# Ledicia/Molecular-Dynamics-Simulation---Lennard-Jones-monoatomic-fluid

Measured on AMD Instinct MI355X. Metric: md_steps_per_sec_n262144_fp64, higher is better.
Workload: dtype f64

## Files before the change

molecular-dynamics-simulation---lennard-jones-monoatomic-fluid_amd/csrc/ljmd_common.cpp:

```cpp
#include "ljmd_common.h"
#include "ljmd_internal.h"

#include <algorithm>
#include <cstdio>
#include <cstring>
#include <limits>

namespace ljmdh {

using namespace ljmdk;

thread_local std::string g_last_error = "";

int failv(std::string *handle_err, int code, const char *fmt, va_list ap)
{
    char buf[512];
    vsnprintf(buf, sizeof buf, fmt, ap);
    g_last_error = buf;
    if (handle_err) *handle_err = buf;
    return code;
}

int check_sim_params(const char *who, int n, double box_length, double dt, double rc)
{
// ... 13 lines not shown
        return fail(nullptr, LJMD_ERR_NO_DEVICE, "%s: no HIP device available (this library has no CPU path)", who);
    if (device < 0 || device >= ndev)
        return fail(nullptr, LJMD_ERR_INVALID_ARG, "%s: device %d out of range (0..%d)", who, device, ndev - 1);
    return LJMD_OK;
}

SimParams derive_params(int n, double box_length, double dt, double rc)
{
    SimParams p;
    p.L = box_length;
    p.invL = 1.0 / box_length;
    p.volume = box_length * box_length * box_length;
    p.rc = rc;
    p.rc2 = rc * rc;
    p.dt = dt;
    p.dt_half = 0.5 * dt;
    p.dt_sq_half = p.dt_half * dt;
    {
        const double npd = (double)n;
        const double rc3 = (rc * rc) * rc;
        const double rc6 = ((rc * rc) * (rc * rc)) * (rc * rc);
        const double tf = 8.0 * kPi * (npd * npd) / (p.volume * rc3);
        p.tail_e = tf * ((1.0 / (3.0 * rc6)) - 1.0) / 3.0;
        p.tail_d = 2.0 * tf * (-2.0 / (3.0 * rc6) + 1.0);
        p.tail_dd = 2.0 * tf * (26.0 / (3.0 * rc6) - 7.0);
    }
    return p;
}

Knobs read_knobs()
{
    auto flag = [](const char *name, bool dflt) { return env_int(name, dflt ? 1 : 0) != 0; };
    auto is = [](const char *name, const char *value) {
        const char *v = std::getenv(name);
        return v && std::strcmp(v, value) == 0;
    };
    auto opt_int = [](const char *name) -> std::optional<int> {
        const char *v = std::getenv(name);
        if (v && *v) return std::atoi(v);
        return std::nullopt;
    };
    Knobs k;
    k.sort = flag("LJMD_SORT", k.sort);
    k.force_generic = flag("LJMD_FORCE_GENERIC", k.force_generic);
    k.force_collectives = flag("LJMD_FORCE_COLLECTIVES", k.force_collectives);
    k.fuse = flag("LJMD_FUSE", k.fuse);
    k.fuse_tail = flag("LJMD_FUSE_TAIL", k.fuse_tail);
    k.fuse_defer_record = flag("LJMD_FUSE_DEFER_RECORD", k.fuse_defer_record);
    k.xcd_remap = std::max(0, env_int("LJMD_N3_XCD_REMAP", k.xcd_remap));
    k.inject_failure_at_step = env_int("LJMD_INJECT_FAILURE_AT_STEP", k.inject_failure_at_step);
    k.exchange_alltoall = is("LJMD_FORCE_EXCHANGE", "alltoall");
    k.resort_every = opt_int("LJMD_RESORT_EVERY");
    k.kd_sort_cub = is("LJMD_KD_SORT", "cub");
    k.n3_row_tiles = env_int("LJMD_N3_ROW_TILES", k.n3_row_tiles);
    k.n3_wg_waves = env_int("LJMD_N3_WG_WAVES", k.n3_wg_waves);
    k.slab_budget_gb = std::max(1, env_int("LJMD_SLAB_BUDGET_GB", k.slab_budget_gb));
    k.n3_both_ties = flag("LJMD_N3_BOTH_TIES", k.n3_both_ties);
    k.n3_min_n = env_int("LJMD_N3_MIN_N", k.n3_min_n);
    k.n3 = flag("LJMD_N3", k.n3);
    k.n3_target_waves = opt_int("LJMD_N3_TARGET_WAVES");
    k.n3_clusters = flag("LJMD_N3_CLUSTERS", k.n3_clusters);
    k.n3_pertile = flag("LJMD_N3_PERTILE", k.n3_pertile);
    k.reduce_split = opt_int("LJMD_REDUCE_SPLIT");
    if (k.reduce_split) k.reduce_split = std::max(0, *k.reduce_split);
    k.walk_chunk = opt_int("LJMD_WALK_CHUNK");
    k.vanhove_chunk = opt_int("LJMD_VANHOVE_CHUNK");
    k.fp32_far_stream = flag("LJMD_FP32_FAR_STREAM", k.fp32_far_stream);
    k.fp32_vfar = flag("LJMD_FP32_VFAR", k.fp32_vfar);
    {
        const char *rs = std::getenv("LJMD_FP32_SPLIT");
        if (rs && *rs) k.fp32_split = std::max(0.0, std::atof(rs));
    }
    k.overlap_exchange = flag("LJMD_OVERLAP_EXCHANGE", k.overlap_exchange);
    k.migrate_blocks = is("LJMD_MIGRATE_DEAL", "blocks");
    {
        const char *xm = std::getenv("LJMD_MULTI_EXCHANGE");
        k.multi_exchange = xm ? xm : "";
    }
    k.multi_migrate_every = std::max(0, env_int("LJMD_MULTI_MIGRATE_EVERY", k.multi_migrate_every));
    k.multi_threads = flag("LJMD_MULTI_THREADS", k.multi_threads);
    k.batch_group_streams = !is("LJMD_BATCH_GROUP_STREAMS", "0");
    return k;
}

void scalars_from_sums(double s12, double s6, double kx, double ky, double kz, double te, double td, double tdd,
                       double *epot, double *ekin, double *d_epot, double *dd_epot)
{
    if (epot) *epot = 4.0 * (s12 - s6) + te;
    if (d_epot) *d_epot = 24.0 * (-2.0 * s12 + s6) + td;
    if (dd_epot) *dd_epot = 24.0 * (26.0 * s12 - 7.0 * s6) + tdd;
    if (ekin) *ekin = 0.5 * (kx + ky + kz);
}

namespace {
void neg192(uint64_t (&x)[3])
{
    x[0] = ~x[0]; x[1] = ~x[1]; x[2] = ~x[2];
    const uint64_t one[3] = {1, 0, 0};
    add192(x, one);
}

void scale192(uint64_t (&x)[3], uint64_t k)
{
    unsigned __int128 carry = 0;
    for (int w = 0; w < 3; ++w) {
        const unsigned __int128 p = (unsigned __int128)x[w] * k + carry;
// ... 50 lines not shown
```

molecular-dynamics-simulation---lennard-jones-monoatomic-fluid_amd/csrc/ljmd_common.h:

```cpp
#ifndef LJMD_COMMON_H
#define LJMD_COMMON_H

#include "ljmd.h"

#include <hip/hip_runtime.h>

#include <cstdarg>
#include <cstddef>
#include <cstdint>
#include <cstdlib>
#include <optional>
#include <string>

namespace ljmdh {

extern thread_local std::string g_last_error;

constexpr double kPi = 3.1415926535897932384626433832795;

int failv(std::string *handle_err, int code, const char *fmt, va_list ap);

inline int fail(std::nullptr_t, int code, const char *fmt, ...)
{
    va_list ap;
// ... 20 lines not shown
    failv(h ? &const_cast<H *>(h)->err : nullptr, code, fmt, ap);
    va_end(ap);
    return code;
}

#define LJMD_HIP(h, call)                                                                   \
    do {                                                                                    \
        hipError_t e_ = (call);                                                             \
        if (e_ != hipSuccess)                                                               \
            return ljmdh::fail((h), LJMD_ERR_HIP, "%s failed: %s (%s:%d)", #call,           \
                               hipGetErrorString(e_), __FILE__, __LINE__);                  \
    } while (0)

#define LJMD_TRY(expr)                      \
    do {                                    \
        const int rc__ = (expr);            \
        if (rc__ != LJMD_OK) return rc__;   \
    } while (0)

inline int env_int(const char *name, int dflt)
{
    const char *v = std::getenv(name);
    return (v && *v) ? std::atoi(v) : dflt;
}

int check_sim_params(const char *who, int n, double box_length, double dt, double rc);

int probe_device(int device, const char *who);

struct SimParams {
    double L = 0, invL = 0, volume = 0, rc = 0, rc2 = 0, dt = 0, dt_half = 0, dt_sq_half = 0;
    double tail_e = 0, tail_d = 0, tail_dd = 0;
};
SimParams derive_params(int n, double box_length, double dt, double rc);

void scalars_from_sums(double s12, double s6, double kx, double ky, double kz, double te, double td, double tdd,
                       double *epot, double *ekin, double *d_epot, double *dd_epot);

void scalars_from_exact_sums(const uint64_t (&ordered)[5][3], double te, double td, double tdd, bool have_e, bool have_k,
                             double *epot, double *ekin, double *d_epot, double *dd_epot);

struct Knobs {
    bool sort = true;
    bool force_generic = false;
    bool force_collectives = false;
    bool fuse = true;
    bool fuse_tail = true;
    bool fuse_defer_record = true;
    int xcd_remap = 4;
    int inject_failure_at_step = -1;
    bool exchange_alltoall = false;
    std::optional<int> resort_every;
    bool kd_sort_cub = false;
    int n3_row_tiles = 0;
    int n3_wg_waves = 0;
    int slab_budget_gb = 64;
    bool n3_both_ties = true;
    int n3_min_n = 4096;
    bool n3 = true;
    std::optional<int> n3_target_waves;
    bool n3_clusters = true;
    bool n3_pertile = true;
    std::optional<int> reduce_split;
    std::optional<int> walk_chunk;
    std::optional<int> vanhove_chunk;
    bool fp32_far_stream = true;
    bool fp32_vfar = true;
    double fp32_split = 5.0;
    bool overlap_exchange = true;
    bool migrate_blocks = false;
    std::string multi_exchange;
    int multi_migrate_every = 2000;
    bool multi_threads = true;
    bool batch_group_streams = true;
};
Knobs read_knobs();

}
#endif
```

molecular-dynamics-simulation---lennard-jones-monoatomic-fluid_amd/csrc/ljmd_engine.cpp:

```cpp
#include "ljmd_engine.h"

namespace ljmdh {

bool fast_path_ok(const ljmd_t *h) { return h->plan.rc_allows_fast && h->positions_compact && !h->knobs.force_generic; }

double *wg_part_now(ljmd_t *h) { return h->d_wg_part + (h->plan.fuse_tail ? (size_t)h->fold_parity * h->wg_part_stride : 0); }

PairArgs pair_args(ljmd_t *h, bool fast)
{
    PairArgs a;
    a.pos = h->d_pos;
    a.slab = h->d_slab;
    a.wg_part = wg_part_now(h);
    a.mask = h->d_mask;
    a.bbox = h->d_bbox;
    a.inline_mask = (fast && h->plan.fuse_tail && !h->plan.use_n3) ? 1 : 0;
    a.rc2_skin = h->rc2 * (1.0 + 1e-10);
    a.n = h->n;
    a.S = h->plan.S;
    a.P = h->plan.P;
    a.G = h->G;
    a.rank = h->rank;
    a.TB = h->plan.TB;
    a.T = h->plan.T;
// ... 97 lines not shown
{
    ReduceArgs a;
    a.slab = h->d_slab;
    a.slab_j = n3 ? h->d_slab_j : nullptr;
    a.flag_j = n3 ? h->d_flag_j : nullptr;
    a.slab_j2 = (n3 && h->mode == LJMD_PRECISION_FP32_FORCE) ? reinterpret_cast<const float *>(h->d_slab_j2) : nullptr;
    a.flag_j2 = (n3 && h->mode == LJMD_PRECISION_FP32_FORCE) ? h->d_flag_j2 : nullptr;
    a.fpart = h->d_fpart;
    a.nslab = nslab;
    a.P = h->plan.P;
    a.G = h->G;
    a.rank = h->rank;
    a.TB = h->plan.TB;
    a.CS = h->plan.CS;
    a.CS2 = h->plan.CS2;
    a.RT = h->plan.rt;
    a.partial = h->d_red_part;
    a.c_split = h->plan.split_s1;
    a.j_split = h->plan.split_j1;
    return a;
}

FinalizeArgs finalize_args(ljmd_t *h, int n_wg, bool with_ke, double pair_scale)
{
    FinalizeArgs a;
    a.pair_scale = pair_scale;
    a.wg_part = wg_part_now(h);
    a.ke_part = h->d_ke_part;
    a.ke_tile = nullptr;
    a.ring = h->d_ring;
    a.ring_pos = h->d_ring_pos;
    a.n_wg = n_wg;
    a.n_ke = with_ke ? h->plan.n_ke : 0;
    a.ring_cap = kRingCap;
    return a;
}

EventSet *next_events(ljmd_t *h)
{
    if (!h->profiling || h->ev_used >= (size_t)kMaxProfiledLaunches) return nullptr;
    if (h->ev_used == h->ev_pool.size()) {
        EventSet q;
        for (auto &e : q.e)
            if (hipEventCreate(&e) != hipSuccess) return nullptr;
        h->ev_pool.push_back(q);
    }
    EventSet *q = &h->ev_pool[h->ev_used++];
    q->has_pos_x = q->has_force_x = false;
    return q;
}

int resort(ljmd_t *h, bool with_accel)
{
    if (!launch_kd_finish || !launch_gather_state)
        return fail(h, LJMD_ERR_HIP, "resort: this build holds no launch_kd_finish / launch_gather_state (ljmd_sort.h)");
    const int levels = (int)h->plan.kd_level_nseg.size(), from = h->plan.kd_finish_from;
    int *cur = h->d_idx, *nxt = h->d_idx2;
    LJMD_HIP(h, launch_iota(cur, h->plan.P, h->stream));
    if (from > 0) LJMD_HIP(h, launch_iota(nxt, h->plan.P, h->stream));
    for (int l = 0; l < from; ++l) {
        const double *axis = own_block(h) + (size_t)h->kd_axis[l] * h->plan.P;
        LJMD_HIP(h, kd_level(h->d_cub, h->cub_bytes, axis, h->L, h->d_kd_keys, h->d_kd_keys2, cur, nxt, h->plan.S,
                             h->plan.kd_level_nseg[l], h->d_kd_offsets + h->plan.kd_level_off[l], h->stream));
        std::swap(cur, nxt);
    }
    for (int l = from; l < levels; l += kKdFinishMaxLevels) {
        KdFinishArgs ka;
        ka.pos = own_block(h);
        ka.P = h->plan.P;
        ka.scale = (double)(1u << kCoordBits) / h->L;
        ka.idx_in = ka.idx_out = cur;
        ka.offsets = h->d_kd_offsets;
        ka.nlevels = std::min(kKdFinishMaxLevels, levels - l);
        for (int k = 0; k < ka.nlevels; ++k) {
            ka.nseg[k] = h->plan.kd_level_nseg[l + k];
            ka.off[k] = (int)h->plan.kd_level_off[l + k];
            ka.axis[k] = h->kd_axis[l + k];
        }
        LJMD_HIP(h, launch_kd_finish(ka, h->stream));
    }
    GatherStateArgs g;
    double *sets[4] = {own_block(h), h->d_ru, h->d_v, with_accel ? h->d_a : nullptr};
    double *outs[4] = {h->d_tmp3, h->d_ru2, h->d_v2, h->d_a2};
    for (int k = 0; k < 4; ++k) {
        g.src[k] = sets[k];
        g.dst[k] = outs[k];
    }
    g.perm = h->d_perm;
    g.perm_out = h->d_perm2;
    g.idx = cur;
    g.P = h->plan.P;
    LJMD_HIP(h, launch_gather_state(g, h->stream));
    LJMD_HIP(h, hipMemcpyAsync(own_block(h), h->d_tmp3, 3 * (size_t)h->plan.P * sizeof(double), hipMemcpyDeviceToDevice,
                               h->stream));
    std::swap(h->d_ru, h->d_ru2);
    std::swap(h->d_v, h->d_v2);
    if (with_accel) std::swap(h->d_a, h->d_a2);
    std::swap(h->d_perm, h->d_perm2);
    h->perm_dirty = true;
    h->steps_since_sort = 0;
    return LJMD_OK;
}

int refresh_perm(ljmd_t *h)
{
    if (!h->perm_dirty) return LJMD_OK;
    LJMD_HIP(h, hipMemcpyAsync(h->h_perm.data(), h->d_perm, (size_t)h->plan.P * sizeof(int), hipMemcpyDeviceToHost,
                               h->stream));
    LJMD_HIP(h, hipStreamSynchronize(h->stream));
    h->perm_dirty = false;
    return LJMD_OK;
}

bool use_comm_stream(const ljmd_t *h) { return h->knobs.overlap_exchange && h->comm_stream != nullptr; }
// ... 363 lines not shown
```

molecular-dynamics-simulation---lennard-jones-monoatomic-fluid_amd/csrc/ljmd_engine.h:

```cpp
#ifndef LJMD_ENGINE_H
#define LJMD_ENGINE_H

#include "ljmd_common.h"

#include <rccl/rccl.h>

#include <algorithm>
#include <cmath>
#include <cstdio>
#include <cstring>
#include <limits>
#include <mutex>
#include <vector>

#include "ljmd_internal.h"
#include "ljmd_resident.h"
#include "ljmd_sort.h"

using namespace ljmdk;

namespace ljmdh {

constexpr unsigned kRingCap = 4096;
constexpr int kTargetWorkgroups = 2048;
constexpr int kXcdMinGroups = 256;
constexpr int kMixedMinN = 16384;
constexpr long kN3ItemsFor4 = 6000;
constexpr long kN3ItemsFor2 = 1000;
constexpr long kN3LargeItems = 131072;
constexpr int kN3MidTargetItems = 32768;
constexpr int kBothTiesMaxGroups = 128;
constexpr int kFuseTailMaxRowTiles = 2;
constexpr int kFuseTailMaxN = 20000;
constexpr int kReduceSplitMinN = 131072;
constexpr int kReduceSplitShare = 8;
constexpr int kMaxProfiledLaunches = 4096;
constexpr int kEventsPerLaunch = 9;

struct EventSet {
    hipEvent_t e[kEventsPerLaunch];
    bool has_pos_x = false, has_force_x = false;
};

struct LaunchPlan {
    int S = 0, P = 0;
    int TB = 0, T = 0, W = 0;
    bool rc_allows_fast = false;
    bool sort_enabled = true;
    int resort_every = 20;
    std::vector<int> kd_level_nseg;
    std::vector<size_t> kd_level_off;
    std::vector<int> kd_offsets;
    int kd_finish_from = 0;
    int nslab_g = 1, chunk_g = 0;
    int nslab_t = 1, chunk_t = 0;
    bool use_n3 = false;
    int wg_waves = 1;
    bool both_ties = false;
    int uchunk = 0;
    int CS = 0, CS2 = 0, j_by_group = 0;
    int NG = 0, NGo = 0, Dmax = 0, nslab_n = 1, dchunk = 0;
    int rt = kRowTiles;
    bool fuse_tail = false;
    int split_s1 = 0, split_j1 = 0;
    int nslab_max = 1, n_wg_max = 0;
    int n_ke = 0;
};

int plan_engine(const SimParams &sim, int n, int n_ranks, int precision_mode, const Knobs &k, LaunchPlan *out);

}

struct ljmd_multi;

using namespace ljmdh;

struct ljmd : ljmdh::SimParams {
    ljmd_multi *multi = nullptr;
    bool poisoned = false;
    int inject_failure_at = -1;
    int n = 0, rank = 0, G = 1, device = 0, mode = 0;
    ljmdh::Knobs knobs;
    ljmdh::LaunchPlan plan;
    bool tail_on = true;
    bool positions_compact = false;
    bool positions_wide = false;
    bool have_state = false, have_accel = false;
    int steps_since_sort = 0;

    hipStream_t stream = nullptr;
    ncclComm_t comm = nullptr;
    hipStream_t comm_stream = nullptr;
    hipEvent_t ev_pos_ready = nullptr, ev_gather_done = nullptr;
    bool gather_done_for_step = false;
    double *d_pos = nullptr;
    double *d_ru = nullptr, *d_v = nullptr, *d_a = nullptr;
    double *d_slab = nullptr;
    double *d_wg_part = nullptr;
    double *d_fold = nullptr;
    unsigned *d_ticket = nullptr;
    bool want_energy = true;
    int kick_hint = -1;
    bool next_drift_hint = false;
    bool reduce_deferred = false, deferred_n3 = false;
    int deferred_nslab = 0;
    bool drift_prefused = false;
    double *d_ke_tile = nullptr;
    bool boxes_valid = false;
    double *d_ke_part = nullptr;
    double *d_ring = nullptr;
    int rec_stride = kPartialStride;
    __int128 *d_fslab = nullptr;
    unsigned *d_fflag = nullptr;
    int64_t *d_fblk = nullptr;
    int64_t *d_frec = nullptr;
    bool pending_energy = true;
    unsigned *d_ring_pos = nullptr;
    double *d_bbox = nullptr;
    uint64_t *d_mask = nullptr;
    double *d_pos_tc = nullptr;
    unsigned *d_desc = nullptr;
    unsigned *d_desc_far = nullptr;
    float *d_desc2 = nullptr;
    int *d_idx = nullptr, *d_idx2 = nullptr, *d_perm = nullptr, *d_perm2 = nullptr;
    double *d_tmp3 = nullptr;
    double *d_ru2 = nullptr, *d_v2 = nullptr, *d_a2 = nullptr;
    void *d_cub = nullptr;
    size_t cub_bytes = 0;
    std::vector<int> kd_axis;
    int *d_kd_offsets = nullptr;
    unsigned long long *d_kd_keys = nullptr, *d_kd_keys2 = nullptr;

    unsigned ring_consumed = 0;
    unsigned ring_issued = 0;
    bool fold_pending = false;
    ljmdk::FinalizeArgs pending_fold{};
    int fold_parity = 0;
    size_t wg_part_stride = 0;
    double *d_slab_j = nullptr;
    unsigned char *d_flag_j = nullptr;
    double *d_red_part = nullptr;
    hipStream_t side_stream = nullptr;
    hipEvent_t ev_side_go = nullptr, ev_side_done = nullptr;
    uint64_t *d_mask_far = nullptr;
    double *d_slab_j2 = nullptr;
    unsigned char *d_flag_j2 = nullptr;
    double *d_fpart = nullptr, *d_frecv = nullptr;
    double *d_fall = nullptr;
    bool forces_pending = false;
    bool external_force_exchange = false;
    int pending_n_wg = 0;
    double pending_scale = 0.5;

    double *h_stage = nullptr;
    double *h_ring = nullptr;
    std::vector<int> h_perm;
    bool perm_dirty = false;

    hipStream_t far_stream = nullptr;
    hipEvent_t ev_far_go = nullptr, ev_far_done = nullptr;
    hipStream_t copy_stream = nullptr;
    hipEvent_t ev_snap_ready = nullptr, ev_snap_done = nullptr;
    double *d_snap = nullptr, *h_snap = nullptr;
    int *d_snap_perm = nullptr, *h_snap_perm = nullptr;
    bool snap_in_flight = false;
    bool snap_ready = false;

    int *d_gid0 = nullptr;
    std::vector<int> h_gid0;
    bool migrated = false;
    double *d_mig = nullptr;
    int *d_mig_idx = nullptr, *d_mig_idx2 = nullptr;
    unsigned long long *d_mig_keys = nullptr, *d_mig_keys2 = nullptr;
    int *d_mig_offsets = nullptr;
    void *d_mig_cub = nullptr;
    size_t mig_cub_bytes = 0;
    std::vector<int> mig_level_nseg, mig_axis;
    std::vector<size_t> mig_level_off;
    double mig_ext[3] = {0, 0, 0};
    int32_t migrations = 0;

    ljmdr::RdfState rdf;
    ljmdt::TcfState tcf;
// ... 59 lines not shown
```

molecular-dynamics-simulation---lennard-jones-monoatomic-fluid_amd/csrc/ljmd_plan.cpp:

```cpp
#include "ljmd_engine.h"

namespace ljmdh {

namespace {
int rt_align(int uchunk, int rt)
{
    int m = 1;
    while ((m * uchunk) % rt != 0) ++m;
    return m;
}
}

int plan_engine(const SimParams &sim, int n, int n_ranks, int precision_mode, const Knobs &k, LaunchPlan *out)
{
    LaunchPlan p;
    p.S = n / n_ranks;
    p.P = ((p.S + kSlotAlign - 1) / kSlotAlign) * kSlotAlign;
    p.TB = p.P / kTile;
    p.T = n_ranks * p.TB;
    p.W = (p.T + 63) / 64;
    p.rc_allows_fast = sim.rc <= (1.0 - 1e-9) * 0.5 * sim.L;
    p.sort_enabled = k.sort && n >= 1024;
    p.resort_every = std::max(1, k.resort_every.value_or(n >= 1000000 ? 5 : n >= 131072 ? 10 : n > 40000 ? 20
                                                              : n > kFuseTailMaxN ? 50 : 200));
    {
        const int tiles = (p.S + kTile - 1) / kTile;
        std::vector<int> bounds = {0, tiles};
        while (true) {
            bool any = false;
            for (size_t j = 0; j + 1 < bounds.size(); ++j) any = any || (bounds[j + 1] - bounds[j] > 1);
            if (!any) break;
            p.kd_level_off.push_back(p.kd_offsets.size());
            p.kd_level_nseg.push_back((int)bounds.size() - 1);
            for (int b : bounds) p.kd_offsets.push_back(std::min(b * kTile, p.S));
            std::vector<int> next;
            for (size_t j = 0; j + 1 < bounds.size(); ++j) {
                next.push_back(bounds[j]);
                const int t = bounds[j + 1] - bounds[j];
                if (t > 1) next.push_back(bounds[j] + (t + 1) / 2);
            }
            next.push_back(tiles);
            bounds.swap(next);
        }
        const int levels = (int)p.kd_level_nseg.size();
        p.kd_finish_from = levels;
        for (int l = levels - 1; l >= 0 && !k.kd_sort_cub; --l) {
            int largest = 0;
            for (int j = 0; j < p.kd_level_nseg[l]; ++j)
                largest = std::max(largest, p.kd_offsets[p.kd_level_off[l] + j + 1] - p.kd_offsets[p.kd_level_off[l] + j]);
            if (largest > kKdFinishCap) break;
            p.kd_finish_from = l;
        }
    }

    const int row_blocks = p.P / kBlock;
    {
        int ns = (kTargetWorkgroups + row_blocks - 1) / row_blocks;
        ns = std::max(1, std::min(ns, (n + 63) / 64));
        p.chunk_g = ((n + ns - 1) / ns + 7) / 8 * 8;
        p.nslab_g = (n + p.chunk_g - 1) / p.chunk_g;
    }
    {
        int ns = (kTargetWorkgroups + row_blocks - 1) / row_blocks;
        ns = std::max(1, std::min(ns, p.T));
        p.chunk_t = (p.T + ns - 1) / ns;
        p.nslab_t = (p.T + p.chunk_t - 1) / p.chunk_t;
    }
    {
        const bool mixed_mode = precision_mode == LJMD_PRECISION_FP32_FORCE;
        int rt = k.n3_row_tiles;
        if (mixed_mode) rt = kRowTiles;
        if (rt != 1 && rt != 2 && rt != kRowTiles) {
            auto items = [&](int cand) { const long ngo = p.TB / cand; return ngo * ((long)n_ranks * ngo / 2 + 1); };
            rt = items(kRowTiles) >= kN3ItemsFor4 ? kRowTiles : items(2) >= kN3ItemsFor2 ? 2 : 1;
        }
        p.rt = rt;
        p.NGo = p.TB / rt;
        p.NG = n_ranks * p.NGo;
        p.Dmax = p.NG / 2;
        int wg = k.n3_wg_waves;
        if (wg != 1 && wg != 2 && wg != 4) {
            const double budget = 1e9 * k.slab_budget_gb;
            const double full = (double)p.T * (n_ranks > 1 ? p.NGo : p.Dmax + 1) * 3.0 * kTile * sizeof(double);
            wg = full <= budget ? 1 : full <= 2.0 * budget ? 2 : 4;
        }
        if (rt != kRowTiles || p.NGo < 16 * wg) wg = 1;
        p.wg_waves = wg;
        p.both_ties = wg == 1 && n_ranks == 1 && !mixed_mode && p.NG <= kBothTiesMaxGroups && k.n3_both_ties;
        p.j_by_group = (n_ranks > 1 || p.NG % wg != 0) ? 1 : 0;
        p.CS = p.j_by_group ? (p.NGo + wg - 1) / wg : (p.Dmax + wg - 1) / wg + 1;
        p.CS2 = n_ranks > 1 ? p.NGo : p.Dmax + 1;
        p.use_n3 = k.n3 && n >= k.n3_min_n && (n_ranks == 1 || p.rc_allows_fast) &&
                   precision_mode != LJMD_PRECISION_FP64_REPRODUCIBLE;
        const int n_off = p.Dmax + p.wg_waves;
        const int n_units = n_off * rt;
        const bool plenty = (long)p.NGo * n_off >= kN3LargeItems || n_ranks > 1;
        const int target_waves = std::max(1, k.n3_target_waves.value_or(plenty ? 131072 : kN3MidTargetItems));
        const int ns_wanted = (target_waves + p.NGo - 1) / p.NGo;
        int ns = std::max(1, std::min(ns_wanted, n_off));
        const bool small_single = n_ranks == 1 && n <= kFuseTailMaxN && rt <= kFuseTailMaxRowTiles;
        const int ns_cap = small_single ? std::max(1, kDirectFoldMax / std::max(1, p.NGo)) : n_units;
        ns = std::min(ns, ns_cap);
        p.dchunk = (n_off + ns - 1) / ns;
        p.uchunk = p.dchunk * rt;
// ... 33 lines not shown
```

molecular-dynamics-simulation---lennard-jones-monoatomic-fluid_amd/csrc/ljmd_sort.h:

```cpp
#ifndef LJMD_SORT_H
#define LJMD_SORT_H

#include <hip/hip_runtime.h>

namespace ljmdk {

constexpr int kCoordBits = 24;

constexpr int kKdFinishCap = 4096;
constexpr int kKdFinishMaxLevels = 6;
constexpr int kKdFinishBlock = 1024;

struct KdFinishArgs {
    const double *pos = nullptr;
    int P = 0;
    double scale = 0.0;
    const int *idx_in = nullptr;
    int *idx_out = nullptr;
    const int *offsets = nullptr;
    int nlevels = 0;
    int nseg[kKdFinishMaxLevels] = {};
    int off[kKdFinishMaxLevels] = {};
    int axis[kKdFinishMaxLevels] = {};
};

struct GatherStateArgs {
    const double *src[4] = {};
    double *dst[4] = {};
    const int *perm = nullptr;
    int *perm_out = nullptr;
    const int *idx = nullptr;
    int P = 0;
};

__attribute__((weak)) hipError_t launch_kd_finish(const KdFinishArgs &a, hipStream_t s);
__attribute__((weak)) hipError_t launch_gather_state(const GatherStateArgs &a, hipStream_t s);

}
#endif
```

molecular-dynamics-simulation---lennard-jones-monoatomic-fluid_amd/csrc/ljmd_sort.hip:

```cpp
#include <hip/hip_runtime.h>
#include <hipcub/hipcub.hpp>

#include "ljmd_internal.h"
#include "ljmd_sort.h"

namespace ljmdk {

__global__ __launch_bounds__(kBlock) void gather_state_kernel(GatherStateArgs g)
{
    const int i = blockIdx.x * kBlock + threadIdx.x;
    if (i >= g.P) return;
    const int s = g.idx[i];
#pragma unroll
    for (int q = 0; q < 4; ++q) {
        if (g.src[q] == nullptr) continue;
#pragma unroll
        for (int k = 0; k < 3; ++k) g.dst[q][(size_t)k * g.P + i] = g.src[q][(size_t)k * g.P + s];
    }
    g.perm_out[i] = g.perm[s];
}


__device__ __forceinline__ unsigned long long kd_quant(double coord, double scale)
{
    const double x = coord * scale;
    return (unsigned long long)fmin(fmax(x, 0.0), (double)((1u << kCoordBits) - 1));
}

__global__ __launch_bounds__(kBlock) void kd_keys_kernel(const double *coord, const int *idx, unsigned long long *keys,
                                                         const int *seg_offsets, int nseg, int S, double scale)
{
    const int i = blockIdx.x * kBlock + threadIdx.x;
    if (i >= S) return;
    int lo = 0, hi = nseg;
    while (hi - lo > 1) {
        const int mid = (lo + hi) >> 1;
        if (seg_offsets[mid] <= i) lo = mid; else hi = mid;
    }
    keys[i] = ((unsigned long long)lo << kCoordBits) | kd_quant(coord[idx[i]], scale);
}

__global__ __launch_bounds__(kBlock) void iota_kernel(int *idx, int P)
{
    const int i = blockIdx.x * kBlock + threadIdx.x;
    if (i < P) idx[i] = i;
}

size_t kd_temp_bytes(int count)
{
    size_t bytes = 0;
    (void)hipcub::DeviceRadixSort::SortPairs(nullptr, bytes, (const unsigned long long *)nullptr,
                                             (unsigned long long *)nullptr, (const int *)nullptr, (int *)nullptr,
                                             count, 0, 64, nullptr);
    return bytes;
}

hipError_t launch_iota(int *idx, int P, hipStream_t s)
{
    hipLaunchKernelGGL(iota_kernel, dim3((P + kBlock - 1) / kBlock), dim3(kBlock), 0, s, idx, P);
    return hipGetLastError();
}

hipError_t kd_level(void *temp, size_t temp_bytes, const double *coord_axis, double L, unsigned long long *keys,
                    unsigned long long *keys_out, int *idx, int *idx_out, int S, int nseg, const int *seg_offsets,
                    hipStream_t s)
{
    hipLaunchKernelGGL(kd_keys_kernel, dim3((S + kBlock - 1) / kBlock), dim3(kBlock), 0, s, coord_axis, idx, keys,
                       seg_offsets, nseg, S, (double)(1u << kCoordBits) / L);
    hipError_t e = hipGetLastError();
    if (e != hipSuccess) return e;
    int segbits = 1;
    while ((1 << segbits) < nseg) ++segbits;
    return hipcub::DeviceRadixSort::SortPairs(temp, temp_bytes, keys, keys_out, idx, idx_out, S, 0,
                                              kCoordBits + segbits, s);
}


__device__ __forceinline__ int last_at_most(const int *b, int n, int x)
{
    int lo = 0, hi = n;
    while (hi - lo > 1) {
        const int mid = (lo + hi) >> 1;
        if (b[mid] <= x) lo = mid; else hi = mid;
    }
    return lo;
}

__device__ __forceinline__ void order_pair(unsigned long long &x, unsigned long long &y, bool up)
{
    if ((x > y) == up) {
        const unsigned long long t = x;
        x = y;
        y = t;
    }
}

__global__ __launch_bounds__(kKdFinishBlock) void kd_finish_kernel(KdFinishArgs a)
{
    constexpr int kMaxSub = kKdFinishCap / kTile;
    __shared__ unsigned long long s_word[kKdFinishCap];
    __shared__ int s_idx[kKdFinishCap];
    __shared__ int s_bound[kKdFinishMaxLevels][kMaxSub + 1];
    __shared__ int s_first[kKdFinishMaxLevels], s_last[kKdFinishMaxLevels];
    const int tid = threadIdx.x;
    const int lo = a.offsets[a.off[0] + blockIdx.x], len = a.offsets[a.off[0] + blockIdx.x + 1] - lo;
    if (len <= 0 || len > kKdFinishCap) return;
    int npad = kTile;
    while (npad < len) npad <<= 1;
    for (int p = tid; p < len; p += kKdFinishBlock) s_idx[p] = a.idx_in[lo + p];
    if (tid < kKdFinishMaxLevels) s_first[tid] = s_last[tid] = 0;
    __syncthreads();
    for (int l = 0; l < a.nlevels; ++l)
        for (int j = tid; j <= a.nseg[l]; j += kKdFinishBlock) {
            const int b = a.offsets[a.off[l] + j];
            if (b == lo) s_first[l] = j;
            if (b == lo + len) s_last[l] = j;
        }
    __syncthreads();
    for (int l = 0; l < a.nlevels; ++l) {
        const int nsub = min(s_last[l] - s_first[l], kMaxSub);
        if (tid <= nsub) s_bound[l][tid] = a.offsets[a.off[l] + s_first[l] + tid] - lo;
    }
    __syncthreads();
    for (int l = 0; l < a.nlevels; ++l) {
        const int nsub = min(s_last[l] - s_first[l], kMaxSub);
        const double *coord = a.pos + (size_t)a.axis[l] * a.P;
        for (int p = tid; p < npad; p += kKdFinishBlock) {
            unsigned long long w = ~0ull;
            if (p < len) {
                const unsigned home = l == 0 ? (unsigned)p : (unsigned)(s_word[p] & 0xffffu);
                const int sub = last_at_most(s_bound[l], nsub, p);
                w = ((unsigned long long)sub << 56) | (kd_quant(coord[s_idx[home]], a.scale) << 32) |
                    ((unsigned long long)p << 16) | home;
            }
            s_word[p] = w;
        }
        __syncthreads();
        for (int k = 2; k <= npad; k <<= 1) {
            int j = k >> 1;
            for (; j >= 2; j >>= 2) {
                const int h = j >> 1;
                for (int t = tid; t < (npad >> 2); t += kKdFinishBlock) {
                    const int i = ((t & ~(h - 1)) << 2) | (t & (h - 1));
                    const bool up = (i & k) == 0;
                    unsigned long long w0 = s_word[i], w1 = s_word[i | h], w2 = s_word[i | j], w3 = s_word[i | j | h];
                    order_pair(w0, w2, up);
                    order_pair(w1, w3, up);
                    order_pair(w0, w1, up);
                    order_pair(w2, w3, up);
                    s_word[i] = w0;
                    s_word[i | h] = w1;
                    s_word[i | j] = w2;
                    s_word[i | j | h] = w3;
                }
                __syncthreads();
            }
            if (j == 1) {
                for (int t = tid; t < (npad >> 1); t += kKdFinishBlock) {
                    const int i = t << 1;
                    unsigned long long w0 = s_word[i], w1 = s_word[i | 1];
                    order_pair(w0, w1, (i & k) == 0);
                    s_word[i] = w0;
                    s_word[i | 1] = w1;
                }
                __syncthreads();
            }
        }
    }
    for (int p = tid; p < len; p += kKdFinishBlock) a.idx_out[lo + p] = s_idx[s_word[p] & 0xffffu];
}

hipError_t launch_kd_finish(const KdFinishArgs &a, hipStream_t s)
{
    if (a.nlevels < 1 || a.nlevels > kKdFinishMaxLevels) return hipErrorInvalidValue;
    hipLaunchKernelGGL(kd_finish_kernel, dim3(a.nseg[0]), dim3(kKdFinishBlock), 0, s, a);
    return hipGetLastError();
}

__global__ __launch_bounds__(kBlock) void iota_blocked_kernel(int *idx, int n, int S, int P)
{
    const int k = blockIdx.x * kBlock + threadIdx.x;
    if (k < n) idx[k] = (k / S) * P + k % S;
}

__global__ __launch_bounds__(kBlock) void kd_keys_blocked_kernel(const double *pos, int axis, int P, const int *idx,
                                                                 unsigned long long *keys, const int *seg_offsets, int nseg,
                                                                 int n, double scale)
{
    const int i = blockIdx.x * kBlock + threadIdx.x;
    if (i >= n) return;
    int lo = 0, hi = nseg;
    while (hi - lo > 1) {
        const int mid = (lo + hi) >> 1;
        if (seg_offsets[mid] <= i) lo = mid; else hi = mid;
    }
    const int st = idx[i], g = st / P, sl = st - g * P;
    keys[i] = ((unsigned long long)lo << kCoordBits) | kd_quant(pos[(size_t)g * 3 * P + (size_t)axis * P + sl], scale);
}

__global__ __launch_bounds__(kBlock) void migrate_pack_kernel(const double *ru, const double *v, const double *a,
                                                              const int *perm, const int *gid0, double *block, int S, int P)
{
    const int s = blockIdx.x * kBlock + threadIdx.x;
    if (s >= P) return;
#pragma unroll
    for (int k = 0; k < 3; ++k) {
        block[(size_t)k * P + s] = ru[(size_t)k * P + s];
        block[(size_t)(3 + k) * P + s] = v[(size_t)k * P + s];
        block[(size_t)(6 + k) * P + s] = a[(size_t)k * P + s];
    }
    const int o = perm[s];
    block[(size_t)9 * P + s] = (s < S && o < S) ? (double)gid0[o] : -1.0;
}

__global__ __launch_bounds__(kBlock) void migrate_select_kernel(const double *pos_all, const double *mig_all, const int *mine,
                                                                double *new_pos, double *ru, double *v, double *a, int *gid0,
                                                                int S, int P)
{
    const int j = blockIdx.x * kBlock + threadIdx.x;
    if (j >= P) return;
    if (j >= S) {
#pragma unroll
        for (int k = 0; k < 3; ++k) {
            new_pos[(size_t)k * P + j] = __builtin_nan("");
            ru[(size_t)k * P + j] = __builtin_nan("");
            v[(size_t)k * P + j] = 0.0;
            a[(size_t)k * P + j] = 0.0;
        }
        gid0[j] = -1;
// ... 70 lines not shown
```

molecular-dynamics-simulation---lennard-jones-monoatomic-fluid_amd/csrc/ljmd_storage.cpp:

```cpp
#include "ljmd_engine.h"

namespace ljmdh {

int allocate_engine(ljmd_t *h)
{
    const bool mixed = h->mode == LJMD_PRECISION_FP32_FORCE;
    const std::vector<int> &kd = h->plan.kd_offsets;
    LJMD_HIP(h, hipSetDevice(h->device));
    LJMD_HIP(h, hipStreamCreateWithFlags(&h->stream, hipStreamNonBlocking));
    const size_t P3 = 3 * (size_t)h->plan.P * sizeof(double);
    LJMD_HIP(h, hipMalloc(&h->d_pos, P3 * h->G));
    LJMD_HIP(h, hipMalloc(&h->d_ru, P3));
    LJMD_HIP(h, hipMalloc(&h->d_v, P3));
    LJMD_HIP(h, hipMalloc(&h->d_a, P3));
    LJMD_HIP(h, hipMalloc(&h->d_tmp3, P3));
    if (h->plan.sort_enabled) {
        LJMD_HIP(h, hipMalloc(&h->d_ru2, P3));
        LJMD_HIP(h, hipMalloc(&h->d_v2, P3));
        LJMD_HIP(h, hipMalloc(&h->d_a2, P3));
    }
    LJMD_HIP(h, hipMalloc(&h->d_slab, P3 * h->plan.nslab_max));
    h->wg_part_stride = 2 * (size_t)h->plan.n_wg_max;
    LJMD_HIP(h, hipMalloc(&h->d_wg_part, (h->plan.fuse_tail ? 2 : 1) * h->wg_part_stride * sizeof(double)));
    if (h->plan.use_n3) {
// ... 13 lines not shown
        LJMD_HIP(h, hipStreamCreateWithPriority(&h->side_stream, hipStreamNonBlocking, least));
        LJMD_HIP(h, hipEventCreateWithFlags(&h->ev_side_go, hipEventDisableTiming));
        LJMD_HIP(h, hipEventCreateWithFlags(&h->ev_side_done, hipEventDisableTiming));
    }
    if (mixed && h->knobs.fp32_far_stream) {
        LJMD_HIP(h, hipStreamCreateWithFlags(&h->far_stream, hipStreamNonBlocking));
        LJMD_HIP(h, hipEventCreateWithFlags(&h->ev_far_go, hipEventDisableTiming));
        LJMD_HIP(h, hipEventCreateWithFlags(&h->ev_far_done, hipEventDisableTiming));
    }
    if (mixed) {
        LJMD_HIP(h, hipMalloc(&h->d_mask_far, (size_t)h->plan.TB * h->plan.W * sizeof(uint64_t)));
        LJMD_HIP(h, hipMalloc(&h->d_desc_far, (size_t)h->plan.NGo * h->plan.T * sizeof(unsigned)));
        const size_t n_blk2 = (size_t)h->plan.T * h->plan.CS2;
        LJMD_HIP(h, hipMalloc(&h->d_slab_j2, n_blk2 * 3 * kTile * sizeof(float)));
        LJMD_HIP(h, hipMalloc(&h->d_flag_j2, n_blk2));
        LJMD_HIP(h, hipMemsetAsync(h->d_flag_j2, 0, n_blk2, h->stream));
    }
    LJMD_HIP(h, hipMalloc(&h->d_fpart, P3 * (needs_force_exchange(h) ? h->G : 1)));
    if (needs_force_exchange(h)) LJMD_HIP(h, hipMalloc(&h->d_frecv, P3));
    if (needs_force_exchange(h) && h->knobs.exchange_alltoall) LJMD_HIP(h, hipMalloc(&h->d_fall, P3 * h->G));
    LJMD_HIP(h, hipMalloc(&h->d_ke_part, 3 * (size_t)h->plan.n_ke * sizeof(double)));
    LJMD_HIP(h, hipMalloc(&h->d_fold, 2 * (size_t)kFoldBlocks * sizeof(double)));
    LJMD_HIP(h, hipMalloc(&h->d_ticket, sizeof(unsigned)));
    LJMD_HIP(h, hipMemsetAsync(h->d_ticket, 0, sizeof(unsigned), h->stream));
    if (h->plan.fuse_tail) {
        LJMD_HIP(h, hipMalloc(&h->d_ke_tile, 2 * 3 * (size_t)h->plan.T * sizeof(double)));
        LJMD_HIP(h, hipMemsetAsync(h->d_ke_tile, 0, 2 * 3 * (size_t)h->plan.T * sizeof(double), h->stream));
    }
    if (reproducible(h)) {
        h->rec_stride = kExactWords;
        LJMD_HIP(h, hipMalloc(&h->d_fslab, (size_t)h->plan.nslab_t * kFixedQuantities * h->plan.P * sizeof(__int128)));
        LJMD_HIP(h, hipMalloc(&h->d_fflag, (size_t)h->plan.nslab_t * h->plan.TB * sizeof(unsigned)));
        LJMD_HIP(h, hipMalloc(&h->d_fblk, (size_t)(h->plan.P / kBlock) * kExactWords * sizeof(int64_t)));
        LJMD_HIP(h, hipMalloc(&h->d_frec, kExactWords * sizeof(int64_t)));
    }
    LJMD_HIP(h, hipMalloc(&h->d_ring, (size_t)kRingCap * h->rec_stride * sizeof(double)));
    LJMD_HIP(h, hipMalloc(&h->d_ring_pos, sizeof(unsigned)));
    LJMD_HIP(h, hipMalloc(&h->d_bbox, (size_t)h->plan.T * kBoxStride * sizeof(double)));
    LJMD_HIP(h, hipMalloc(&h->d_mask, (size_t)h->plan.TB * h->plan.W * sizeof(uint64_t)));
    LJMD_HIP(h, hipMalloc(&h->d_idx, (size_t)h->plan.P * sizeof(int)));
    LJMD_HIP(h, hipMalloc(&h->d_idx2, (size_t)h->plan.P * sizeof(int)));
    LJMD_HIP(h, hipMalloc(&h->d_perm, (size_t)h->plan.P * sizeof(int)));
    LJMD_HIP(h, hipMalloc(&h->d_perm2, (size_t)h->plan.P * sizeof(int)));
    LJMD_HIP(h, hipMalloc(&h->d_gid0, (size_t)h->plan.P * sizeof(int)));
    LJMD_HIP(h, launch_iota_offset(h->d_gid0, h->plan.S, h->plan.P, h->rank * h->plan.S, h->stream));
    h->cub_bytes = kd_temp_bytes(h->plan.S);
    LJMD_HIP(h, hipMalloc(&h->d_cub, std::max<size_t>(h->cub_bytes, 16)));
    LJMD_HIP(h, hipMalloc(&h->d_kd_keys, (size_t)h->plan.P * sizeof(unsigned long long)));
    LJMD_HIP(h, hipMalloc(&h->d_kd_keys2, (size_t)h->plan.P * sizeof(unsigned long long)));
    LJMD_HIP(h, hipMalloc(&h->d_kd_offsets, std::max<size_t>(kd.size(), 2) * sizeof(int)));
    if (!kd.empty())
        LJMD_HIP(h, hipMemcpyAsync(h->d_kd_offsets, kd.data(), kd.size() * sizeof(int),
                                   hipMemcpyHostToDevice, h->stream));
    LJMD_HIP(h, hipMemsetAsync(h->d_ring_pos, 0, sizeof(unsigned), h->stream));
    LJMD_HIP(h, hipMemsetAsync(h->d_a, 0, P3, h->stream));
    LJMD_HIP(h, hipMemsetAsync(h->d_ke_part, 0, 3 * (size_t)h->plan.n_ke * sizeof(double), h->stream));
    LJMD_HIP(h, hipHostMalloc(&h->h_stage, P3 * std::max(h->G, 4), hipHostMallocDefault));
    LJMD_HIP(h, hipHostMalloc(&h->h_ring, (size_t)kRingCap * h->rec_stride * sizeof(double),
                              hipHostMallocDefault));
    LJMD_HIP(h, hipStreamSynchronize(h->stream));
    return LJMD_OK;
}

void release(ljmd_t *h)
{
    if (!h) return;
    if (h->device >= 0) (void)hipSetDevice(h->device);
    if (h->stream) (void)hipStreamSynchronize(h->stream);
    release_resident(h);
    if (h->comm_stream) (void)hipStreamSynchronize(h->comm_stream);
    if (h->comm) (void)ncclCommDestroy(h->comm);
    if (h->comm_stream) (void)hipStreamDestroy(h->comm_stream);
    if (h->far_stream) {
        (void)hipStreamSynchronize(h->far_stream);
        (void)hipStreamDestroy(h->far_stream);
    }
    if (h->side_stream) {
        (void)hipStreamSynchronize(h->side_stream);
        (void)hipStreamDestroy(h->side_stream);
    }
    if (h->ev_side_go) (void)hipEventDestroy(h->ev_side_go);
    if (h->ev_side_done) (void)hipEventDestroy(h->ev_side_done);
    if (h->ev_far_go) (void)hipEventDestroy(h->ev_far_go);
    if (h->ev_far_done) (void)hipEventDestroy(h->ev_far_done);
    if (h->ev_pos_ready) (void)hipEventDestroy(h->ev_pos_ready);
    if (h->ev_gather_done) (void)hipEventDestroy(h->ev_gather_done);
    for (auto &q : h->ev_pool)
        for (auto &e : q.e) (void)hipEventDestroy(e);
    void *dev[] = {h->d_pos, h->d_ru, h->d_v, h->d_a, h->d_slab, h->d_wg_part, h->d_ke_part, h->d_ring,
                   h->d_ring_pos, h->d_bbox, h->d_mask, h->d_idx, h->d_idx2,
                   h->d_perm, h->d_perm2, h->d_tmp3, h->d_ru2, h->d_v2, h->d_a2, h->d_cub, h->d_slab_j, h->d_flag_j, h->d_fpart, h->d_frecv, h->d_fall,
                   h->d_kd_offsets, h->d_kd_keys, h->d_kd_keys2, h->d_mask_far, h->d_slab_j2, h->d_flag_j2, h->d_fold, h->d_ticket,
                   h->d_desc, h->d_desc_far, h->d_desc2, h->d_red_part, h->d_ke_tile, h->d_pos_tc, h->d_gid0, h->d_mig, h->d_mig_idx, h->d_mig_idx2, h->d_mig_keys,
                   h->d_mig_keys2, h->d_mig_offsets, h->d_mig_cub, h->d_fslab, h->d_fflag, h->d_fblk, h->d_frec};
    for (void *p : dev) (void)hipFree(p);
    if (h->h_stage) (void)hipHostFree(h->h_stage);
    if (h->h_ring) (void)hipHostFree(h->h_ring);
    if (h->copy_stream) {
        (void)hipStreamSynchronize(h->copy_stream);
        (void)hipStreamDestroy(h->copy_stream);
    }
    if (h->ev_snap_ready) (void)hipEventDestroy(h->ev_snap_ready);
    if (h->ev_snap_done) (void)hipEventDestroy(h->ev_snap_done);
    if (h->d_snap) (void)hipFree(h->d_snap);
    if (h->d_snap_perm) (void)hipFree(h->d_snap_perm);
    if (h->h_snap) (void)hipHostFree(h->h_snap);
    if (h->h_snap_perm) (void)hipHostFree(h->h_snap_perm);
    if (h->stream) (void)hipStreamDestroy(h->stream);
    delete h;
}

int download_state(ljmd_t *h, double *const dsts[12], unsigned n_records)
{
    const size_t P = h->plan.P;
    const double *srcs[4] = {own_block(h), h->d_ru, h->d_v, h->d_a};
    bool want[4];
    for (int w = 0; w < 4; ++w) {
        want[w] = dsts[3 * w] || dsts[3 * w + 1] || dsts[3 * w + 2];
        if (want[w])
            LJMD_HIP(h, hipMemcpyAsync(h->h_stage + (size_t)w * 3 * P, srcs[w], 3 * P * sizeof(double),
                                       hipMemcpyDeviceToHost, h->stream));
    }
    if (h->perm_dirty)
        LJMD_HIP(h, hipMemcpyAsync(h->h_perm.data(), h->d_perm, P * sizeof(int), hipMemcpyDeviceToHost, h->stream));
    if (n_records > 0) {
        const int rc_ = fetch_ring(h, n_records);
        if (rc_ != LJMD_OK) return rc_;
    } else {
        LJMD_HIP(h, hipStreamSynchronize(h->stream));
    }
    h->perm_dirty = false;
    for (int w = 0; w < 4; ++w) {
        if (!want[w]) continue;
        for (int k = 0; k < 3; ++k) {
            double *dst = dsts[3 * w + k];
            if (!dst) continue;
            const double *st = h->h_stage + ((size_t)w * 3 + k) * P;
            for (int i = 0; i < h->plan.P; ++i) {
                const int o = h->h_perm[i];
                if (o < h->plan.S) dst[o] = st[i];
            }
        }
    }
    return LJMD_OK;
}
// ... 34 lines not shown
```

Before: 57.37.

## Replace CUB segmented sort in upper k-d levels with chunked bitonic plus merge passes

Result: no change. 57.37, median of 3 (-0.0%).

```diff
diff --git a/molecular-dynamics-simulation---lennard-jones-monoatomic-fluid_amd/csrc/ljmd_common.cpp b/molecular-dynamics-simulation---lennard-jones-monoatomic-fluid_amd/csrc/ljmd_common.cpp
--- a/molecular-dynamics-simulation---lennard-jones-monoatomic-fluid_amd/csrc/ljmd_common.cpp
+++ b/molecular-dynamics-simulation---lennard-jones-monoatomic-fluid_amd/csrc/ljmd_common.cpp
@@ -89,6 +89,7 @@
     k.exchange_alltoall = is("LJMD_FORCE_EXCHANGE", "alltoall");
     k.resort_every = opt_int("LJMD_RESORT_EVERY");
     k.kd_sort_cub = is("LJMD_KD_SORT", "cub");
+    k.kd_sort_finish = is("LJMD_KD_SORT", "finish");
     k.n3_row_tiles = env_int("LJMD_N3_ROW_TILES", k.n3_row_tiles);
     k.n3_wg_waves = env_int("LJMD_N3_WG_WAVES", k.n3_wg_waves);
     k.slab_budget_gb = std::max(1, env_int("LJMD_SLAB_BUDGET_GB", k.slab_budget_gb));
diff --git a/molecular-dynamics-simulation---lennard-jones-monoatomic-fluid_amd/csrc/ljmd_common.h b/molecular-dynamics-simulation---lennard-jones-monoatomic-fluid_amd/csrc/ljmd_common.h
--- a/molecular-dynamics-simulation---lennard-jones-monoatomic-fluid_amd/csrc/ljmd_common.h
+++ b/molecular-dynamics-simulation---lennard-jones-monoatomic-fluid_amd/csrc/ljmd_common.h
@@ -96,6 +96,7 @@
     bool exchange_alltoall = false;
     std::optional<int> resort_every;
     bool kd_sort_cub = false;
+    bool kd_sort_finish = false;
     int n3_row_tiles = 0;
     int n3_wg_waves = 0;
     int slab_budget_gb = 64;
diff --git a/molecular-dynamics-simulation---lennard-jones-monoatomic-fluid_amd/csrc/ljmd_engine.cpp b/molecular-dynamics-simulation---lennard-jones-monoatomic-fluid_amd/csrc/ljmd_engine.cpp
--- a/molecular-dynamics-simulation---lennard-jones-monoatomic-fluid_amd/csrc/ljmd_engine.cpp
+++ b/molecular-dynamics-simulation---lennard-jones-monoatomic-fluid_amd/csrc/ljmd_engine.cpp
@@ -173,14 +173,34 @@
 
 int resort(ljmd_t *h, bool with_accel)
 {
-    if (!launch_kd_finish || !launch_gather_state)
-        return fail(h, LJMD_ERR_HIP, "resort: this build holds no launch_kd_finish / launch_gather_state (ljmd_sort.h)");
+    if (!launch_kd_merge_level || !launch_kd_finish || !launch_gather_state)
+        return fail(h, LJMD_ERR_HIP,
+                    "resort: this build holds no launch_kd_merge_level / launch_kd_finish / launch_gather_state (ljmd_sort.h)");
     const int levels = (int)h->plan.kd_level_nseg.size(), from = h->plan.kd_finish_from;
+    const bool merge = !h->plan.kd_merge_passes.empty();
     int *cur = h->d_idx, *nxt = h->d_idx2;
     LJMD_HIP(h, launch_iota(cur, h->plan.P, h->stream));
     if (from > 0) LJMD_HIP(h, launch_iota(nxt, h->plan.P, h->stream));
     for (int l = 0; l < from; ++l) {
         const double *axis = own_block(h) + (size_t)h->kd_axis[l] * h->plan.P;
+        if (merge) {
+            KdMergeArgs ma;
+            ma.coord = axis;
+            ma.scale = (double)(1u << kCoordBits) / h->L;
+            ma.idx_in = cur;
+            ma.idx_out = nxt;
+            ma.words = h->d_kd_keys;
+            ma.words2 = h->d_kd_keys2;
+            ma.offsets = h->d_kd_offsets + h->plan.kd_level_off[l];
+            ma.nseg = h->plan.kd_level_nseg[l];
+            ma.S = h->plan.S;
+            ma.chunks = h->d_kd_chunks + h->plan.kd_chunk_off[l];
+            ma.nchunks = h->plan.kd_chunk_n[l];
+            ma.passes = h->plan.kd_merge_passes[l];
+            LJMD_HIP(h, launch_kd_merge_level(ma, h->stream));
+            std::swap(cur, nxt);
+            continue;
+        }
         LJMD_HIP(h, kd_level(h->d_cub, h->cub_bytes, axis, h->L, h->d_kd_keys, h->d_kd_keys2, cur, nxt, h->plan.S,
                              h->plan.kd_level_nseg[l], h->d_kd_offsets + h->plan.kd_level_off[l], h->stream));
         std::swap(cur, nxt);
diff --git a/molecular-dynamics-simulation---lennard-jones-monoatomic-fluid_amd/csrc/ljmd_engine.h b/molecular-dynamics-simulation---lennard-jones-monoatomic-fluid_amd/csrc/ljmd_engine.h
--- a/molecular-dynamics-simulation---lennard-jones-monoatomic-fluid_amd/csrc/ljmd_engine.h
+++ b/molecular-dynamics-simulation---lennard-jones-monoatomic-fluid_amd/csrc/ljmd_engine.h
@@ -52,6 +52,10 @@
     std::vector<size_t> kd_level_off;
     std::vector<int> kd_offsets;
     int kd_finish_from = 0;
+    std::vector<int> kd_chunk_n;
+    std::vector<size_t> kd_chunk_off;
+    std::vector<int> kd_chunks;
+    std::vector<int> kd_merge_passes;
     int nslab_g = 1, chunk_g = 0;
     int nslab_t = 1, chunk_t = 0;
     bool use_n3 = false;
@@ -128,7 +132,7 @@
     void *d_cub = nullptr;
     size_t cub_bytes = 0;
     std::vector<int> kd_axis;
-    int *d_kd_offsets = nullptr;
+    int *d_kd_offsets = nullptr, *d_kd_chunks = nullptr;
     unsigned long long *d_kd_keys = nullptr, *d_kd_keys2 = nullptr;
 
     unsigned ring_consumed = 0;
diff --git a/molecular-dynamics-simulation---lennard-jones-monoatomic-fluid_amd/csrc/ljmd_plan.cpp b/molecular-dynamics-simulation---lennard-jones-monoatomic-fluid_amd/csrc/ljmd_plan.cpp
--- a/molecular-dynamics-simulation---lennard-jones-monoatomic-fluid_amd/csrc/ljmd_plan.cpp
+++ b/molecular-dynamics-simulation---lennard-jones-monoatomic-fluid_amd/csrc/ljmd_plan.cpp
@@ -50,6 +50,19 @@
                 largest = std::max(largest, p.kd_offsets[p.kd_level_off[l] + j + 1] - p.kd_offsets[p.kd_level_off[l] + j]);
             if (largest > kKdFinishCap) break;
             p.kd_finish_from = l;
+        }
+        for (int l = 0; l < p.kd_finish_from && !k.kd_sort_cub && !k.kd_sort_finish; ++l) {
+            p.kd_chunk_off.push_back(p.kd_chunks.size());
+            int largest = 0;
+            for (int j = 0; j < p.kd_level_nseg[l]; ++j) {
+                const int b = p.kd_offsets[p.kd_level_off[l] + j], e = p.kd_offsets[p.kd_level_off[l] + j + 1];
+                for (int c = b; c < e; c += kKdChunk) p.kd_chunks.push_back(c);
+                largest = std::max(largest, e - b);
+            }
+            p.kd_chunk_n.push_back((int)(p.kd_chunks.size() - p.kd_chunk_off.back()));
+            int passes = 0;
+            for (long run = kKdChunk; run < largest; run *= 2) ++passes;
+            p.kd_merge_passes.push_back(passes);
         }
     }
 
diff --git a/molecular-dynamics-simulation---lennard-jones-monoatomic-fluid_amd/csrc/ljmd_sort.h b/molecular-dynamics-simulation---lennard-jones-monoatomic-fluid_amd/csrc/ljmd_sort.h
--- a/molecular-dynamics-simulation---lennard-jones-monoatomic-fluid_amd/csrc/ljmd_sort.h
+++ b/molecular-dynamics-simulation---lennard-jones-monoatomic-fluid_amd/csrc/ljmd_sort.h
@@ -10,6 +10,23 @@
 constexpr int kKdFinishCap = 4096;
 constexpr int kKdFinishMaxLevels = 6;
 constexpr int kKdFinishBlock = 1024;
+
+constexpr int kKdChunk = 2048;
+constexpr int kKdChunkBlock = 512;
+static_assert(kKdChunk <= kKdFinishCap, "a level above the cap needs at least one merge pass: its last pass writes the permutation");
+
+struct KdMergeArgs {
+    const double *coord = nullptr;
+    double scale = 0.0;
+    const int *idx_in = nullptr;
+    int *idx_out = nullptr;
+    unsigned long long *words = nullptr, *words2 = nullptr;
+    const int *offsets = nullptr;
+    int nseg = 0, S = 0;
+    const int *chunks = nullptr;
+    int nchunks = 0;
+    int passes = 0;
+};
 
 struct KdFinishArgs {
     const double *pos = nullptr;
@@ -33,6 +50,7 @@
     int P = 0;
 };
 
+__attribute__((weak)) hipError_t launch_kd_merge_level(const KdMergeArgs &a, hipStream_t s);
 __attribute__((weak)) hipError_t launch_kd_finish(const KdFinishArgs &a, hipStream_t s);
 __attribute__((weak)) hipError_t launch_gather_state(const GatherStateArgs &a, hipStream_t s);
 
diff --git a/molecular-dynamics-simulation---lennard-jones-monoatomic-fluid_amd/csrc/ljmd_sort.hip b/molecular-dynamics-simulation---lennard-jones-monoatomic-fluid_amd/csrc/ljmd_sort.hip
--- a/molecular-dynamics-simulation---lennard-jones-monoatomic-fluid_amd/csrc/ljmd_sort.hip
+++ b/molecular-dynamics-simulation---lennard-jones-monoatomic-fluid_amd/csrc/ljmd_sort.hip
@@ -1,5 +1,7 @@
 #include <hip/hip_runtime.h>
 #include <hipcub/hipcub.hpp>
+
+#include <utility>
 
 #include "ljmd_internal.h"
 #include "ljmd_sort.h"
@@ -92,6 +94,40 @@
         const unsigned long long t = x;
         x = y;
         y = t;
+    }
+}
+
+template <int kThreads> __device__ __forceinline__ void bitonic_sort_lds(unsigned long long *s_word, int npad, int tid)
+{
+    for (int k = 2; k <= npad; k <<= 1) {
+        int j = k >> 1;
+        for (; j >= 2; j >>= 2) {
+            const int h = j >> 1;
+            for (int t = tid; t < (npad >> 2); t += kThreads) {
+                const int i = ((t & ~(h - 1)) << 2) | (t & (h - 1));
+                const bool up = (i & k) == 0;
+                unsigned long long w0 = s_word[i], w1 = s_word[i | h], w2 = s_word[i | j], w3 = s_word[i | j | h];
+                order_pair(w0, w2, up);
+                order_pair(w1, w3, up);
+                order_pair(w0, w1, up);
+                order_pair(w2, w3, up);
+                s_word[i] = w0;
+                s_word[i | h] = w1;
+                s_word[i | j] = w2;
+                s_word[i | j | h] = w3;
+            }
+            __syncthreads();
+        }
+        if (j == 1) {
+            for (int t = tid; t < (npad >> 1); t += kThreads) {
+                const int i = t << 1;
+                unsigned long long w0 = s_word[i], w1 = s_word[i | 1];
+                order_pair(w0, w1, (i & k) == 0);
+                s_word[i] = w0;
+                s_word[i | 1] = w1;
+            }
+            __syncthreads();
+        }
     }
 }
 
@@ -136,36 +172,7 @@
             s_word[p] = w;
         }
         __syncthreads();
-        for (int k = 2; k <= npad; k <<= 1) {
-            int j = k >> 1;
-            for (; j >= 2; j >>= 2) {
-                const int h = j >> 1;
-                for (int t = tid; t < (npad >> 2); t += kKdFinishBlock) {
-                    const int i = ((t & ~(h - 1)) << 2) | (t & (h - 1));
-                    const bool up = (i & k) == 0;
-                    unsigned long long w0 = s_word[i], w1 = s_word[i | h], w2 = s_word[i | j], w3 = s_word[i | j | h];
-                    order_pair(w0, w2, up);
-                    order_pair(w1, w3, up);
-                    order_pair(w0, w1, up);
-                    order_pair(w2, w3, up);
-                    s_word[i] = w0;
-                    s_word[i | h] = w1;
-                    s_word[i | j] = w2;
-                    s_word[i | j | h] = w3;
-                }
-                __syncthreads();
-            }
-            if (j == 1) {
-                for (int t = tid; t < (npad >> 1); t += kKdFinishBlock) {
-                    const int i = t << 1;
-                    unsigned long long w0 = s_word[i], w1 = s_word[i | 1];
-                    order_pair(w0, w1, (i & k) == 0);
-                    s_word[i] = w0;
-                    s_word[i | 1] = w1;
-                }
-                __syncthreads();
-            }
-        }
+        bitonic_sort_lds<kKdFinishBlock>(s_word, npad, tid);
     }
     for (int p = tid; p < len; p += kKdFinishBlock) a.idx_out[lo + p] = s_idx[s_word[p] & 0xffffu];
 }
@@ -175,6 +182,72 @@
     if (a.nlevels < 1 || a.nlevels > kKdFinishMaxLevels) return hipErrorInvalidValue;
     hipLaunchKernelGGL(kd_finish_kernel, dim3(a.nseg[0]), dim3(kKdFinishBlock), 0, s, a);
     return hipGetLastError();
+}
+
+
+__global__ __launch_bounds__(kKdChunkBlock) void kd_chunk_sort_kernel(KdMergeArgs a)
+{
+    __shared__ unsigned long long s_word[kKdChunk];
+    const int tid = threadIdx.x;
+    const int lo = a.chunks[blockIdx.x];
+    const int hi = min(lo + kKdChunk, a.offsets[last_at_most(a.offsets, a.nseg, lo) + 1]);
+    const int len = hi - lo;
+    if (lo < 0 || len <= 0 || hi > a.S) return;
+    int npad = 2;
+    while (npad < len) npad <<= 1;
+    for (int p = tid; p < npad; p += kKdChunkBlock)
+        s_word[p] = p < len ? (kd_quant(a.coord[a.idx_in[lo + p]], a.scale) << 32) | (unsigned)(lo + p) : ~0ull;
+    __syncthreads();
+    bitonic_sort_lds<kKdChunkBlock>(s_word, npad, tid);
+    for (int p = tid; p < len; p += kKdChunkBlock) a.words[lo + p] = s_word[p];
+}
+
+__device__ __forceinline__ int words_below(const unsigned long long *in, int b, int e, unsigned long long w)
+{
+    int lo = b, hi = e;
+    while (lo < hi) {
+        const int mid = (lo + hi) >> 1;
+        if (in[mid] < w) lo = mid + 1; else hi = mid;
+    }
+    return lo - b;
+}
+
+template <bool kLast>
+__global__ __launch_bounds__(kBlock) void kd_merge_pass_kernel(const unsigned long long *in, unsigned long long *out,
+                                                               const int *idx_in, int *idx_out, const int *offsets, int nseg,
+                                                               int S, int run)
+{
+    const int i = blockIdx.x * kBlock + threadIdx.x;
+    if (i >= S) return;
+    const int seg = last_at_most(offsets, nseg, i);
+    const int s0 = offsets[seg], s1 = offsets[seg + 1];
+    const int pair = s0 + (i - s0) / (2 * run) * (2 * run);
+    const int mid = min(pair + run, s1), end = min(mid + run, s1);
+    const unsigned long long w = in[i];
+    const int dest = i < mid ? i + words_below(in, mid, end, w) : pair + (i - mid) + words_below(in, pair, mid, w);
+    if (kLast) idx_out[dest] = idx_in[(unsigned)w];
+    else out[dest] = w;
+}
+
+hipError_t launch_kd_merge_level(const KdMergeArgs &a, hipStream_t s)
+{
+    if (a.passes < 1 || a.nchunks < 1 || a.nseg < 1 || a.S < 1 || a.idx_in == a.idx_out) return hipErrorInvalidValue;
+    hipLaunchKernelGGL(kd_chunk_sort_kernel, dim3(a.nchunks), dim3(kKdChunkBlock), 0, s, a);
+    hipError_t e = hipGetLastError();
+    const dim3 grid((a.S + kBlock - 1) / kBlock);
+    unsigned long long *in = a.words, *out = a.words2;
+    int run = kKdChunk;
+    for (int p = 0; p < a.passes && e == hipSuccess; ++p, run *= 2) {
+        if (p + 1 < a.passes)
+            hipLaunchKernelGGL(kd_merge_pass_kernel<false>, grid, dim3(kBlock), 0, s, in, out, a.idx_in, a.idx_out, a.offsets,
+                               a.nseg, a.S, run);
+        else
+            hipLaunchKernelGGL(kd_merge_pass_kernel<true>, grid, dim3(kBlock), 0, s, in, out, a.idx_in, a.idx_out, a.offsets,
+                               a.nseg, a.S, run);
+        e = hipGetLastError();
+        std::swap(in, out);
+    }
+    return e;
 }
 
 __global__ __launch_bounds__(kBlock) void iota_blocked_kernel(int *idx, int n, int S, int P)
diff --git a/molecular-dynamics-simulation---lennard-jones-monoatomic-fluid_amd/csrc/ljmd_storage.cpp b/molecular-dynamics-simulation---lennard-jones-monoatomic-fluid_amd/csrc/ljmd_storage.cpp
--- a/molecular-dynamics-simulation---lennard-jones-monoatomic-fluid_amd/csrc/ljmd_storage.cpp
+++ b/molecular-dynamics-simulation---lennard-jones-monoatomic-fluid_amd/csrc/ljmd_storage.cpp
@@ -89,6 +89,11 @@
     if (!kd.empty())
         LJMD_HIP(h, hipMemcpyAsync(h->d_kd_offsets, kd.data(), kd.size() * sizeof(int),
                                    hipMemcpyHostToDevice, h->stream));
+    if (!h->plan.kd_chunks.empty()) {
+        LJMD_HIP(h, hipMalloc(&h->d_kd_chunks, h->plan.kd_chunks.size() * sizeof(int)));
+        LJMD_HIP(h, hipMemcpyAsync(h->d_kd_chunks, h->plan.kd_chunks.data(), h->plan.kd_chunks.size() * sizeof(int),
+                                   hipMemcpyHostToDevice, h->stream));
+    }
     LJMD_HIP(h, hipMemsetAsync(h->d_ring_pos, 0, sizeof(unsigned), h->stream));
     LJMD_HIP(h, hipMemsetAsync(h->d_a, 0, P3, h->stream));
     LJMD_HIP(h, hipMemsetAsync(h->d_ke_part, 0, 3 * (size_t)h->plan.n_ke * sizeof(double), h->stream));
@@ -127,7 +132,7 @@
     void *dev[] = {h->d_pos, h->d_ru, h->d_v, h->d_a, h->d_slab, h->d_wg_part, h->d_ke_part, h->d_ring,
                    h->d_ring_pos, h->d_bbox, h->d_mask, h->d_idx, h->d_idx2,
                    h->d_perm, h->d_perm2, h->d_tmp3, h->d_ru2, h->d_v2, h->d_a2, h->d_cub, h->d_slab_j, h->d_flag_j, h->d_fpart, h->d_frecv, h->d_fall,
-                   h->d_kd_offsets, h->d_kd_keys, h->d_kd_keys2, h->d_mask_far, h->d_slab_j2, h->d_flag_j2, h->d_fold, h->d_ticket,
+                   h->d_kd_offsets, h->d_kd_chunks, h->d_kd_keys, h->d_kd_keys2, h->d_mask_far, h->d_slab_j2, h->d_flag_j2, h->d_fold, h->d_ticket,
                    h->d_desc, h->d_desc_far, h->d_desc2, h->d_red_part, h->d_ke_tile, h->d_pos_tc, h->d_gid0, h->d_mig, h->d_mig_idx, h->d_mig_idx2, h->d_mig_keys,
                    h->d_mig_keys2, h->d_mig_offsets, h->d_mig_cub, h->d_fslab, h->d_fflag, h->d_fblk, h->d_frec};
     for (void *p : dev) (void)hipFree(p);
```
